# BrByte/brb_framework

Measured on AMD Instinct MI355X. Metric: GiB/s (device-resident) + Mrecords/s over 1500B buffers at 1/2/4/8 MI355X, higher is better.
Workload: dtype u32

## Files before the change

brb_framework_amd/__init__.py:

```python
from .crypto import (
    BATCH_ALL_DEVICES,
    BATCH_DROPPED,
    TRANSFORM_DROPPED,
    TestOption,
    test_option,
    async_fault_check,
    BATCH_ASYNC,
    BATCH_DEVICE,
    BATCH_HOST,
    BRB_BLOWFISH_CTX,
    BRB_MD5_CTX,
    BRB_RC4_State,
    RC4_STATE_BYTES,
    RC4MD5_HEADER,
    BrbSha1Ctx,
    LIB_PATH,
    CRYPTO_FUNC_RC4,
    CRYPTO_FUNC_RC4_MD5,
    OP_READ,
    OP_WRITE,
    TransformBatcher,
    HostRegion,
    BATCHER_ZERO_COPY,
    BATCHER_PIPELINED,
# ... 54 lines not shown
    sha1_final_batch,
    md5_update_segments_batch,
    sha1_update_segments_batch,
    md5_update_segments_lower_batch,
    md5_lower_text_batch,
    MD5_CTX_BYTES,
    SHA1_CTX_BYTES,
    md5_ctx_init,
    md5_ctx_update,
    md5_ctx_update_lower,
    md5_ctx_final,
    sha1_ctx_init,
    sha1_ctx_update,
    sha1_ctx_final,
    fixed_route,
    FIXED_ROUTE_LANE_A4,
    FIXED_ROUTE_LANE_ANY,
    FIXED_ROUTE_LINE,
    FIXED_ROUTE_VAR_LINE,
    FIXED_ROUTE_DMA_TICKET,
    FIXED_ROUTE_B64R_8,
    FIXED_ROUTE_B64R_4,
    FIXED_ROUTE_B64,
    FIXED_ROUTE_DMA_SHORT,
)

__all__ = [
    "BATCH_ASYNC", "BATCH_DEVICE", "BATCH_HOST", "BRB_BLOWFISH_CTX", "BRB_MD5_CTX", "BrbSha1Ctx",
    "LIB_PATH", "blowfish_ctx_bytes", "blowfish_decrypt_batch", "blowfish_encrypt_batch",
    "blowfish_init", "exported_symbols", "gpu_available", "lib", "md5_batch", "md5_batch_fixed",
    "sha1_batch", "sha1_batch_fixed", "BRB_RC4_State", "RC4_STATE_BYTES", "RC4MD5_HEADER", "rc4_crypt_batch",
    "rc4_init", "rc4_state_bytes", "rc4_states", "rc4md5_frame_batch", "rc4md5_open_batch", "rc4_crypt_list_batch",
    "rc4md5_frame_list_batch", "rc4md5_open_list_batch", "BATCHER_CONN_LISTS",
    "rc4_mixed_list_batch", "BATCHER_MIXED", "RC4_KIND_CRYPT", "RC4_KIND_FRAME", "RC4_KIND_OPEN", "membuf_decrypt",
    "membuf_encrypt", "membuf_key", "membuf_span", "md5_batch_segments", "metadata_pack_batch", "metadata_unpack_batch", "metadata_unpack_items_batch", "METADATA_INFO_DTYPE", "base64_decode_batch",
    "base64_encode_batch", "CRYPTO_FUNC_RC4", "CRYPTO_FUNC_RC4_MD5", "OP_READ", "OP_WRITE", "TransformBatcher",
    "HostRegion", "BATCHER_ZERO_COPY", "BATCHER_PIPELINED", "BATCH_ALL_DEVICES", "device_count",
    "BATCH_DROPPED", "TRANSFORM_DROPPED", "BATCHER_ALL_DEVICES", "TestOption", "test_option", "async_fault_check",
    "rc4_init_batch", "blowfish_init_batch", "pack_keys", "unpack_keys", "BLOWFISH_CTX_BYTES",
    "blowfish_contexts", "blowfish_encrypt_batch_keyed", "blowfish_decrypt_batch_keyed", "membuf_encrypt_batch",
    "membuf_decrypt_batch", "md5_init_batch", "md5_update_batch", "md5_final_batch", "sha1_init_batch",
    "sha1_update_batch", "sha1_final_batch", "md5_update_segments_batch", "sha1_update_segments_batch",
    "md5_update_segments_lower_batch", "md5_lower_text_batch", "md5_ctx_update_lower", "MD5_CTX_BYTES", "SHA1_CTX_BYTES",
    "md5_ctx_init", "md5_ctx_update", "md5_ctx_final", "sha1_ctx_init", "sha1_ctx_update", "sha1_ctx_final",
    "fixed_route", "FIXED_ROUTE_LANE_A4", "FIXED_ROUTE_LANE_ANY", "FIXED_ROUTE_LINE", "FIXED_ROUTE_VAR_LINE",
    "FIXED_ROUTE_DMA_TICKET", "FIXED_ROUTE_B64R_8", "FIXED_ROUTE_B64R_4", "FIXED_ROUTE_B64", "FIXED_ROUTE_DMA_SHORT",
]
```

brb_framework_amd/crypto.py:

```python
from __future__ import annotations

import ctypes
import os
import subprocess

import numpy as np

HERE = os.path.dirname(os.path.abspath(__file__))
LIB_PATH = os.environ.get("BRB_CRYPTO_LIB") or os.path.join(HERE, "libbrb_crypto_gpu.so")
HEADER_PATH = os.path.join(os.path.dirname(HERE), "include", "brb_crypto.h")

BATCH_HOST = 0x0
BATCH_DEVICE = 0x1
BATCH_ASYNC = 0x2
BATCH_ALL_DEVICES = 0x4
BATCH_DROPPED = -2
BATCH_PARTIAL = -3
BATCH_FAULT = -4
TRANSFORM_DROPPED = -1

u8p = ctypes.POINTER(ctypes.c_uint8)
ulp = ctypes.POINTER(ctypes.c_ulong)


# ... 163 lines not shown
     [ctypes.c_void_p, ctypes.c_uint32, ctypes.c_int, ctypes.c_void_p, ctypes.c_int]),
    ("BRB_TransformBatcherEnableBatchAlgo", ctypes.c_int,
     [ctypes.c_void_p, ctypes.c_void_p, ctypes.c_uint64, ctypes.c_void_p, ctypes.c_void_p, ctypes.c_void_p,
      ctypes.c_void_p]),
    ("BRB_TransformBatcherDisable", ctypes.c_int, [ctypes.c_void_p, ctypes.c_uint32]),
    ("BRB_TransformBatcherRead", ctypes.c_int, [ctypes.c_void_p, ctypes.c_uint32, ctypes.c_void_p, ctypes.c_uint32]),
    ("BRB_TransformBatcherWrite", ctypes.c_int,
     [ctypes.c_void_p, ctypes.c_uint32, ctypes.c_void_p, ctypes.c_uint32, ctypes.c_uint64]),
    ("BRB_TransformBatcherFlush", ctypes.c_int64, [ctypes.c_void_p, ctypes.c_void_p, ctypes.c_void_p]),
    ("BRB_TransformBatcherFlushAsync", ctypes.c_int64, [ctypes.c_void_p, ctypes.c_void_p, ctypes.c_void_p]),
    ("BRB_TransformBatcherGetState", ctypes.c_int,
     [ctypes.c_void_p, ctypes.c_uint32, ctypes.c_int, ctypes.POINTER(BRB_RC4_State)]),
    ("BRB_TransformBatcherInjectFault", ctypes.c_int, [ctypes.c_void_p, ctypes.c_int]),
    ("BRB_CryptoGPU_TestOption", ctypes.c_int, [ctypes.c_char_p, ctypes.c_int, ctypes.POINTER(ctypes.c_int)]),
    ("BRB_CryptoGPU_TestFixedRoute", ctypes.c_int, [ctypes.c_uint64, ctypes.c_uint32]),
    ("BRB_CryptoGPU_HostRegister", ctypes.c_int, [ctypes.c_void_p, ctypes.c_uint64]),
    ("BRB_CryptoGPU_HostUnregister", ctypes.c_int, [ctypes.c_void_p]),
    ("BRB_CryptoGPU_Available", ctypes.c_int, []),
    ("BRB_CryptoGPU_DeviceCount", ctypes.c_int, []),
    ("BRB_CryptoGPU_SetDevice", ctypes.c_int, [ctypes.c_int]),
    ("BRB_CryptoGPU_GetDevice", ctypes.c_int, []),
    ("BRB_CryptoGPU_ThreadCleanup", None, []),
    ("BRB_CryptoGPU_LastError", ctypes.c_char_p, []),
    ("BRB_CryptoGPU_AsyncFaultCheck", ctypes.c_int, []),
    ("BRB_CryptoGPU_Version", ctypes.c_char_p, []),
]


def lib() -> ctypes.CDLL:
    global _LIB
# ... 52 lines not shown
    def __enter__(self):
        self.old = test_option(self.name, self.value)
        return self

    def __exit__(self, *exc):
        test_option(self.name, self.old)
        return False


(FIXED_ROUTE_LANE_A4, FIXED_ROUTE_LANE_ANY, FIXED_ROUTE_LINE, FIXED_ROUTE_VAR_LINE, FIXED_ROUTE_DMA_TICKET,
 FIXED_ROUTE_B64R_8, FIXED_ROUTE_B64R_4, FIXED_ROUTE_B64, FIXED_ROUTE_DMA_SHORT) = range(9)


def fixed_route(addr: int, rec_len: int) -> int:
    return lib().BRB_CryptoGPU_TestFixedRoute(int(addr), int(rec_len))


def _check(rc: int, what: str) -> None:
    if rc != 1:
        msg = lib().BRB_CryptoGPU_LastError().decode(errors="replace")
        raise RuntimeError(f"{what} returned {rc}: {msg}")


def _is_torch(x) -> bool:
    return type(x).__module__.startswith("torch")


def _ptr(x) -> int:
    if x is None:
        return 0
# ... 782 lines not shown
```

brb_framework_amd/csrc/gpu/api_runtime.hip:

```cpp
#include <hip/hip_runtime.h>

#include <algorithm>
#include <atomic>
#include <cstdarg>
#include <cstdio>
#include <cstring>
#include <mutex>
#include <string>
#include <vector>

#include "brb_crypto.h"
#include "api_util.h"
#include "fixed_route.h"
#include "host_pipe.h"
#include "pair_fault.h"
#include "test_options.h"

namespace brb_api {

thread_local std::string t_err;

void clear_err()
{
    t_err.clear();
}

void set_err(const char *fmt, ...)
{
    char buf[512];
    va_list ap;
    va_start(ap, fmt);
// ... 301 lines not shown
            }
            const int prev = brb_opt::g_opt[k.opt].exchange(value, std::memory_order_relaxed);
            if (old)
                *old = prev;
            return BRB_BATCH_OK;
        }
    set_err("unknown test option '%s'", name);
    return BRB_BATCH_BADARG;
}

int BRB_CryptoGPU_TestFixedRoute(uint64_t data_addr, uint32_t rec_len)
{
    return brb_digest::fixed_route(uintptr_t(data_addr), rec_len);
}

}
```

brb_framework_amd/csrc/gpu/digest_var_line.h:

```cpp
#pragma once

#include "byte_stream.h"
#include "digest_line.h"
#include "test_options.h"

namespace brb_digest {

template <class Alg>
BRB_DEV typename Alg::State digest_lane(const uint8_t *a, uint64_t len)
{
    typename Alg::State st = Alg::iv();
    brb_io::BlockSrc src;
    src.init(a, len);
    uint32_t w[16];
    for (uint64_t b = 0; b < (len >> 6); ++b) {
        src.fetch(w);
        Alg::compress(st, w);
    }
    src.fetch(w);
    brb_io::add_marker(w, len);
    Alg::finish(st, w, uint32_t(len & 63), len);
    return st;
}

// ... 9 lines not shown
    for (int m = 32; m >= 1; m >>= 1) {
        const uint64_t o = __shfl_xor(v, m, 64);
        v = o < v ? o : v;
    }
    return v;
}

BRB_DEV uint64_t wave_max64(uint64_t v)
{
#pragma unroll
    for (int m = 32; m >= 1; m >>= 1) {
        const uint64_t o = __shfl_xor(v, m, 64);
        v = o > v ? o : v;
    }
    return v;
}

constexpr uint32_t kSortCG = 4;
constexpr uint32_t kSortNB = 8;

BRB_DEV uint64_t sorted_record(uint64_t g, uint32_t lane, const uint32_t *__restrict__ lens, uint64_t n_rec,
                               uint32_t *scratch)
{
    const uint64_t cg = (g / kSortCG) * kSortCG;
    const uint64_t c0 = cg * 64;
    const uint64_t left = (n_rec + 63) / 64 - cg;
    const uint32_t pc = left < kSortCG ? uint32_t(left) : kSortCG;
    const uint32_t j = uint32_t((g % kSortCG + g / gridDim.x) % pc);
    uint32_t it[kSortCG];
    bool ok[kSortCG];
// ... 75 lines not shown
        return uint64_t(blockIdx.x) + uint64_t(tk) * gridDim.x;
    };
    uint64_t g = uint64_t(blockIdx.x) + uint64_t(wv) * gridDim.x;
    if (g >= n_groups)
        return;
    const uint32_t my_off = wv * 2 * SLOT;
    const uint32_t lds0 = uint32_t(reinterpret_cast<uintptr_t>(ring)) + my_off;
    const uint64_t dbase = reinterpret_cast<uint64_t>(data);
    auto swz = [](uint32_t row) { return (row >> 1) & 7; };

    struct Grp {
        uint64_t a;
        uint64_t r;
        uint32_t len;
        uint32_t K;
        bool line;
        brb_dma::v4i rs;
        uint32_t vq[8];
        uint32_t lq[8];
    };
    const uint64_t first_sorted = brb_first_sorted;
    auto record_of = [&](uint64_t g) -> uint64_t {
        if (SORT && g >= first_sorted && g < n_groups)
            return sorted_record(g, lane, lens, n_rec, sort_scratch + wv * (64 * kSortCG));
        return g * 64 + lane < n_rec ? g * 64 + lane : ~uint64_t(0);
    };
    auto setup = [&](uint64_t g, uint64_t rec, Grp &G) {
        const uint64_t r = rec != ~uint64_t(0) ? rec : uniform64(g * 64);
        G.r = rec;
        G.a = dbase + (FIXED ? r * rec_len : offs[r]);
        G.len = FIXED ? rec_len : (rec != ~uint64_t(0) ? lens[r] : 0u);
        const uint64_t line = G.a & ~uint64_t(127);
        const uint32_t lines = G.len ? uint32_t(((G.a & 127) + G.len + 127) >> 7) : 0u;
        const uint32_t nblk = (G.len >> 6) + ((G.len & 63) ? 1u : 0u);
        const uint64_t lo = uniform64(wave_min64(G.len ? line : ~uint64_t(0)));
        const uint64_t hi = uniform64(wave_max64(G.len ? line + 128 * uint64_t(lines) : 0));
        G.K = __builtin_amdgcn_readfirstlane(uint32_t(wave_max64((nblk + 1) >> 1)));
        G.line = hi > lo && hi - lo < (uint64_t(1) << 31) - (uint64_t(1) << 16);
        const uint64_t base = lo - 4096;
        const uint64_t left = hi - base;
        G.rs.x = __builtin_amdgcn_readfirstlane(int(uint32_t(base)));
        G.rs.y = __builtin_amdgcn_readfirstlane(int(uint32_t(base >> 32) & 0xFFFF));
        G.rs.z = __builtin_amdgcn_readfirstlane(int(left > 0x7FFFFFFFull ? 0x7FFFFFFFu : uint32_t(left)));
        G.rs.w = 0x00020000;
        const uint32_t rel = uint32_t(line - lo);
        const uint32_t l3 = lane >> 3;
        const uint32_t g0 = 16u * ((lane & 7) ^ (l3 >> 1));
#pragma unroll
        for (int q = 0; q < 8; q++) {
            const int src = int(8 * q + l3) * 4;
            const uint32_t rrel = uint32_t(__builtin_amdgcn_ds_bpermute(src, int(rel)));
            G.lq[q] = uint32_t(__builtin_amdgcn_ds_bpermute(src, int(lines)));
            G.vq[q] = (rrel | (q & 1 ? g0 ^ 64u : g0)) + (4096u - 1024u * (q & 3));
        }
    };
    auto issue = [&](Grp &G, uint32_t m, uint32_t slot, bool keep_l2 = false) {
        const uint32_t lm = lds0 + slot * SLOT;
        uint32_t v[8];
#pragma unroll
        for (int q = 0; q < 8; q++)
            v[q] = m < G.lq[q] ? G.vq[q] : OOB;
        uint32_t keep;
#define BRB_VLINE_DMA8(POL)                                                                     \
        asm volatile("s_mov_b32 %0, m0\n\t"                                                    \
                     "s_mov_b32 m0, %10\n\t"                                                   \
                     "s_nop 0\n\t"                                                             \
                     "buffer_load_dwordx4 %1, %9, 0 offen " POL "lds\n\t"                      \
                     "buffer_load_dwordx4 %2, %9, 0 offen offset:1024 " POL "lds\n\t"          \
                     "buffer_load_dwordx4 %3, %9, 0 offen offset:2048 " POL "lds\n\t"          \
                     "buffer_load_dwordx4 %4, %9, 0 offen offset:3072 " POL "lds\n\t"          \
                     "s_mov_b32 m0, %11\n\t"                                                   \
                     "s_nop 0\n\t"                                                             \
                     "buffer_load_dwordx4 %5, %9, 0 offen " POL "lds\n\t"                      \
                     "buffer_load_dwordx4 %6, %9, 0 offen offset:1024 " POL "lds\n\t"          \
                     "buffer_load_dwordx4 %7, %9, 0 offen offset:2048 " POL "lds\n\t"          \
                     "buffer_load_dwordx4 %8, %9, 0 offen offset:3072 " POL "lds\n\t"          \
// ... 15 lines not shown
        G.rs.z = z;
    };
    auto start = [&](Grp &G) {
        if (G.line) {
            issue(G, 0, 0, FIXED);
            issue(G, 1, 1, FIXED);
        }
    };

    uint32_t ae[33], ao[33];
    auto win_setup = [&](const Grp &G) {
        const uint32_t sh4 = uint32_t(G.a) & 124u;
        const uint32_t fr = (my_off + lane * 128) | (swz(lane) << 4);
#pragma unroll
        for (uint32_t i = 0; i < 33; i++) {
            const uint32_t q4 = sh4 + 4 * i;
            ae[i] = ((q4 & 124u) ^ fr) | ((q4 & 128u) << 6);
            ao[i] = ae[i] ^ SLOT;
            asm volatile("" : "+v"(ao[i]));
        }
    };
    uint32_t w0[16], w1[16];
    auto read_window = [&](const uint32_t (&ad)[33], uint32_t fb) {
        uint32_t d[33];
#pragma unroll
        for (int i = 0; i < 33; i++)
            d[i] = *reinterpret_cast<const uint32_t *>(ring + ad[i]);
        __builtin_amdgcn_s_waitcnt(0xC07F);
#pragma unroll
        for (int i = 0; i < 16; i++) {
            w0[i] = __builtin_amdgcn_alignbit(d[i + 1], d[i], fb);
            w1[i] = __builtin_amdgcn_alignbit(d[i + 17], d[i + 16], fb);
// ... 7 lines not shown
    for (;;) {
        const uint64_t gn = take();
        const uint64_t rn = record_of(gn);
        const uint64_t r = G.r;
        typename Alg::State st;
        if (!G.line) {
            st = digest_lane<Alg>(reinterpret_cast<const uint8_t *>(G.a), G.len);
            if (gn < n_groups) {
                setup(gn, rn, Gn);
                start(Gn);
            }
        } else {
            win_setup(G);
            const uint32_t fb = (uint32_t(G.a) & 3u) * 8u;
            const uint32_t nfull = G.len >> 6, t = G.len & 63;
            const uint32_t tb = t ? nfull : 0xFFFFFFFFu;
            uint32_t wt[16];
#pragma unroll
            for (int i = 0; i < 16; i++)
                wt[i] = 0;
            st = Alg::iv();
            const uint32_t K = G.K;
            auto step = [&](uint32_t k, const uint32_t (&ad)[33], uint32_t refill_slot) {
                brb_dma::wait_vmcnt<0>();
                read_window(ad, fb);
                if (k < K) {
                    issue(G, k + 1, refill_slot);
                } else if (gn < n_groups) {
                    setup(gn, rn, Gn);
                    start(Gn);
                }
                const uint32_t b = 2 * k - 2;
                if (b < nfull)
                    Alg::compress(st, w0);
                if (b + 1 < nfull)
                    Alg::compress(st, w1);
                if (__builtin_amdgcn_ballot_w64(tb - b < 2) != 0) {
#pragma unroll
                    for (int i = 0; i < 16; i++)
                        wt[i] = tb == b ? w0[i] : tb == b + 1 ? w1[i] : wt[i];
                }
            };
            if (K == 0) {
                brb_dma::wait_vmcnt<0>();
                if (gn < n_groups) {
                    setup(gn, rn, Gn);
                    start(Gn);
                }
            }
            for (uint32_t k = 1; k <= K; k += 2) {
                step(k, ae, 0);
                if (k == K)
                    break;
                step(k + 1, ao, 1);
            }
            if (t == 0) {
                Alg::pad_only(st, G.len);
            } else {
#pragma unroll
                for (uint32_t i = 0; i < 16; i++) {
                    const uint32_t o = 4 * i;
                    const uint32_t keep = t > o ? (t - o < 4 ? t - o : 4) : 0;
                    uint32_t v = keep == 4 ? wt[i] : wt[i] & ((1u << (8 * keep)) - 1u);
                    if (t >= o && t < o + 4)
                        v |= 0x80u << (8 * (t - o));
                    wt[i] = v;
                }
                Alg::finish(st, wt, t, G.len);
            }
        }
        if (r != ~uint64_t(0))
            Alg::template store<OUT_ALIGNED>(out, r, st);
        g = gn;
        if (g >= n_groups)
            break;
        G = Gn;
    }
}

template <class Alg>
hipError_t launch_var_line(const uint8_t *data, const uint64_t *offs, const uint32_t *lens, uint64_t n_rec, uint8_t *out,
                           bool out_al, hipStream_t s)
{
// ... 37 lines not shown
```

brb_framework_amd/csrc/gpu/md5_device.h:

```cpp
#pragma once

#include "brb_gpu_common.h"

#define BRB_MD5_F1(x, y, z) ((z) ^ ((x) & ((y) ^ (z))))
#define BRB_MD5_F2(x, y, z) ((y) ^ ((z) & ((x) ^ (y))))
#define BRB_MD5_F3(x, y, z) __builtin_amdgcn_bitop3_b32((x), (y), (z), 0x96)
#define BRB_MD5_F4(x, y, z) ((y) ^ ((x) | ~(z)))
#define BRB_MD5_STEP(F, a, b, c, d, m, k, s) (a) = (b) + rotl<s>((a) + F((b), (c), (d)) + ((m) + (k)))

struct Md5State {
    uint32_t a, b, c, d;
};

BRB_DEV Md5State md5_iv()
{
    return Md5State{0x67452301u, 0xefcdab89u, 0x98badcfeu, 0x10325476u};
}

#define BRB_MD5_STEP3X(a, b, c, d, m, k, s)                                               \
    do {                                                                                 \
        const uint32_t x_ = (a) + (m) + (k), cd_ = (c) ^ (d);                            \
        uint32_t f_;                                                                     \
        asm("v_xad_u32 %0, %1, %2, %3" : "=v"(f_) : "v"(b), "v"(cd_), "v"(x_));          \
        (a) = (b) + rotl<s>(f_);                                                         \
    } while (0)

template <bool XAD = true>
BRB_DEV void md5_compress(Md5State &st, const uint32_t (&m)[16])
{
    uint32_t a = st.a, b = st.b, c = st.c, d = st.d;

    BRB_MD5_STEP(BRB_MD5_F1, a, b, c, d, m[0], 0xd76aa478u, 7);
    BRB_MD5_STEP(BRB_MD5_F1, d, a, b, c, m[1], 0xe8c7b756u, 12);
    BRB_MD5_STEP(BRB_MD5_F1, c, d, a, b, m[2], 0x242070dbu, 17);
    BRB_MD5_STEP(BRB_MD5_F1, b, c, d, a, m[3], 0xc1bdceeeu, 22);
    BRB_MD5_STEP(BRB_MD5_F1, a, b, c, d, m[4], 0xf57c0fafu, 7);
    BRB_MD5_STEP(BRB_MD5_F1, d, a, b, c, m[5], 0x4787c62au, 12);
    BRB_MD5_STEP(BRB_MD5_F1, c, d, a, b, m[6], 0xa8304613u, 17);
    BRB_MD5_STEP(BRB_MD5_F1, b, c, d, a, m[7], 0xfd469501u, 22);
    BRB_MD5_STEP(BRB_MD5_F1, a, b, c, d, m[8], 0x698098d8u, 7);
    BRB_MD5_STEP(BRB_MD5_F1, d, a, b, c, m[9], 0x8b44f7afu, 12);
    BRB_MD5_STEP(BRB_MD5_F1, c, d, a, b, m[10], 0xffff5bb1u, 17);
    BRB_MD5_STEP(BRB_MD5_F1, b, c, d, a, m[11], 0x895cd7beu, 22);
    BRB_MD5_STEP(BRB_MD5_F1, a, b, c, d, m[12], 0x6b901122u, 7);
    BRB_MD5_STEP(BRB_MD5_F1, d, a, b, c, m[13], 0xfd987193u, 12);
// ... 5 lines not shown
    BRB_MD5_STEP(BRB_MD5_F2, c, d, a, b, m[11], 0x265e5a51u, 14);
    BRB_MD5_STEP(BRB_MD5_F2, b, c, d, a, m[0], 0xe9b6c7aau, 20);
    BRB_MD5_STEP(BRB_MD5_F2, a, b, c, d, m[5], 0xd62f105du, 5);
    BRB_MD5_STEP(BRB_MD5_F2, d, a, b, c, m[10], 0x02441453u, 9);
    BRB_MD5_STEP(BRB_MD5_F2, c, d, a, b, m[15], 0xd8a1e681u, 14);
    BRB_MD5_STEP(BRB_MD5_F2, b, c, d, a, m[4], 0xe7d3fbc8u, 20);
    BRB_MD5_STEP(BRB_MD5_F2, a, b, c, d, m[9], 0x21e1cde6u, 5);
    BRB_MD5_STEP(BRB_MD5_F2, d, a, b, c, m[14], 0xc33707d6u, 9);
    BRB_MD5_STEP(BRB_MD5_F2, c, d, a, b, m[3], 0xf4d50d87u, 14);
    BRB_MD5_STEP(BRB_MD5_F2, b, c, d, a, m[8], 0x455a14edu, 20);
    BRB_MD5_STEP(BRB_MD5_F2, a, b, c, d, m[13], 0xa9e3e905u, 5);
    BRB_MD5_STEP(BRB_MD5_F2, d, a, b, c, m[2], 0xfcefa3f8u, 9);
    BRB_MD5_STEP(BRB_MD5_F2, c, d, a, b, m[7], 0x676f02d9u, 14);
    BRB_MD5_STEP(BRB_MD5_F2, b, c, d, a, m[12], 0x8d2a4c8au, 20);

    if constexpr (XAD) BRB_MD5_STEP3X(a, b, c, d, m[5], 0xfffa3942u, 4); else BRB_MD5_STEP(BRB_MD5_F3, a, b, c, d, m[5], 0xfffa3942u, 4);
    if constexpr (XAD) BRB_MD5_STEP3X(d, a, b, c, m[8], 0x8771f681u, 11); else BRB_MD5_STEP(BRB_MD5_F3, d, a, b, c, m[8], 0x8771f681u, 11);
    if constexpr (XAD) BRB_MD5_STEP3X(c, d, a, b, m[11], 0x6d9d6122u, 16); else BRB_MD5_STEP(BRB_MD5_F3, c, d, a, b, m[11], 0x6d9d6122u, 16);
    if constexpr (XAD) BRB_MD5_STEP3X(b, c, d, a, m[14], 0xfde5380cu, 23); else BRB_MD5_STEP(BRB_MD5_F3, b, c, d, a, m[14], 0xfde5380cu, 23);
    if constexpr (XAD) BRB_MD5_STEP3X(a, b, c, d, m[1], 0xa4beea44u, 4); else BRB_MD5_STEP(BRB_MD5_F3, a, b, c, d, m[1], 0xa4beea44u, 4);
    if constexpr (XAD) BRB_MD5_STEP3X(d, a, b, c, m[4], 0x4bdecfa9u, 11); else BRB_MD5_STEP(BRB_MD5_F3, d, a, b, c, m[4], 0x4bdecfa9u, 11);
    if constexpr (XAD) BRB_MD5_STEP3X(c, d, a, b, m[7], 0xf6bb4b60u, 16); else BRB_MD5_STEP(BRB_MD5_F3, c, d, a, b, m[7], 0xf6bb4b60u, 16);
    if constexpr (XAD) BRB_MD5_STEP3X(b, c, d, a, m[10], 0xbebfbc70u, 23); else BRB_MD5_STEP(BRB_MD5_F3, b, c, d, a, m[10], 0xbebfbc70u, 23);
    if constexpr (XAD) BRB_MD5_STEP3X(a, b, c, d, m[13], 0x289b7ec6u, 4); else BRB_MD5_STEP(BRB_MD5_F3, a, b, c, d, m[13], 0x289b7ec6u, 4);
    if constexpr (XAD) BRB_MD5_STEP3X(d, a, b, c, m[0], 0xeaa127fau, 11); else BRB_MD5_STEP(BRB_MD5_F3, d, a, b, c, m[0], 0xeaa127fau, 11);
    if constexpr (XAD) BRB_MD5_STEP3X(c, d, a, b, m[3], 0xd4ef3085u, 16); else BRB_MD5_STEP(BRB_MD5_F3, c, d, a, b, m[3], 0xd4ef3085u, 16);
    if constexpr (XAD) BRB_MD5_STEP3X(b, c, d, a, m[6], 0x04881d05u, 23); else BRB_MD5_STEP(BRB_MD5_F3, b, c, d, a, m[6], 0x04881d05u, 23);
    if constexpr (XAD) BRB_MD5_STEP3X(a, b, c, d, m[9], 0xd9d4d039u, 4); else BRB_MD5_STEP(BRB_MD5_F3, a, b, c, d, m[9], 0xd9d4d039u, 4);
    if constexpr (XAD) BRB_MD5_STEP3X(d, a, b, c, m[12], 0xe6db99e5u, 11); else BRB_MD5_STEP(BRB_MD5_F3, d, a, b, c, m[12], 0xe6db99e5u, 11);
    if constexpr (XAD) BRB_MD5_STEP3X(c, d, a, b, m[15], 0x1fa27cf8u, 16); else BRB_MD5_STEP(BRB_MD5_F3, c, d, a, b, m[15], 0x1fa27cf8u, 16);
    if constexpr (XAD) BRB_MD5_STEP3X(b, c, d, a, m[2], 0xc4ac5665u, 23); else BRB_MD5_STEP(BRB_MD5_F3, b, c, d, a, m[2], 0xc4ac5665u, 23);

    BRB_MD5_STEP(BRB_MD5_F4, a, b, c, d, m[0], 0xf4292244u, 6);
    BRB_MD5_STEP(BRB_MD5_F4, d, a, b, c, m[7], 0x432aff97u, 10);
    BRB_MD5_STEP(BRB_MD5_F4, c, d, a, b, m[14], 0xab9423a7u, 15);
    BRB_MD5_STEP(BRB_MD5_F4, b, c, d, a, m[5], 0xfc93a039u, 21);
    BRB_MD5_STEP(BRB_MD5_F4, a, b, c, d, m[12], 0x655b59c3u, 6);
    BRB_MD5_STEP(BRB_MD5_F4, d, a, b, c, m[3], 0x8f0ccc92u, 10);
    BRB_MD5_STEP(BRB_MD5_F4, c, d, a, b, m[10], 0xffeff47du, 15);
    BRB_MD5_STEP(BRB_MD5_F4, b, c, d, a, m[1], 0x85845dd1u, 21);
    BRB_MD5_STEP(BRB_MD5_F4, a, b, c, d, m[8], 0x6fa87e4fu, 6);
    BRB_MD5_STEP(BRB_MD5_F4, d, a, b, c, m[15], 0xfe2ce6e0u, 10);
    BRB_MD5_STEP(BRB_MD5_F4, c, d, a, b, m[6], 0xa3014314u, 15);
    BRB_MD5_STEP(BRB_MD5_F4, b, c, d, a, m[13], 0x4e0811a1u, 21);
    BRB_MD5_STEP(BRB_MD5_F4, a, b, c, d, m[4], 0xf7537e82u, 6);
    BRB_MD5_STEP(BRB_MD5_F4, d, a, b, c, m[11], 0xbd3af235u, 10);
// ... 24 lines not shown
};

BRB_DEV void md5_finish(Md5State &st, uint32_t (&w)[16], uint32_t t, uint64_t total_len)
{
    if (t >= 56) {
        md5_compress(st, w);
#pragma unroll
        for (int i = 0; i < 14; i++)
            w[i] = 0;
    }
    w[14] = uint32_t(total_len << 3);
    w[15] = uint32_t(total_len >> 29);
    md5_compress(st, w);
}

BRB_DEV void md5_pad_only(Md5State &st, uint64_t total_len)
{
    uint32_t w[16] = {0x80u};
    w[14] = uint32_t(total_len << 3);
    w[15] = uint32_t(total_len >> 29);
    md5_compress<false>(st, w);
}
```

brb_framework_amd/csrc/gpu/md5_kernels.hip:

```cpp
#include "brb_kernels.h"
#include "byte_stream.h"
#include "digest_dma.h"
#include "digest_var_line.h"
#include "md5_device.h"

namespace {

struct Md5Alg;

struct Out16 {
    template <bool ALIGNED>
    static BRB_DEV void store(uint8_t *out, uint64_t r, const Md5State &st)
    {
        const uint4 v = make_uint4(st.a, st.b, st.c, st.d);
        if (ALIGNED)
            reinterpret_cast<uint4 *>(out)[r] = v;
        else
            __builtin_memcpy(out + 16 * r, &v, 16);
    }
};

struct Md5Alg {
    using State = Md5State;
    static BRB_DEV State iv() { return md5_iv(); }
    static BRB_DEV void compress(State &st, uint32_t (&w)[16]) { md5_compress(st, w); }
    static BRB_DEV void finish(State &st, uint32_t (&w)[16], uint32_t t, uint64_t len) { md5_finish(st, w, t, len); }
    static BRB_DEV void pad_only(State &st, uint64_t len) { md5_pad_only(st, len); }
    template <bool ALIGNED>
    static BRB_DEV void store(uint8_t *out, uint64_t r, const State &st) { Out16::store<ALIGNED>(out, r, st); }
};

template <int BLOCK, bool OUT_ALIGNED>
__global__ __launch_bounds__(BLOCK) void md5_fixed_a4_kernel(const uint8_t *__restrict__ data, uint32_t rec_len,
                                                              uint64_t n_rec, uint8_t *__restrict__ out)
{
    const uint64_t r = uint64_t(blockIdx.x) * BLOCK + threadIdx.x;
    if (r >= n_rec)
        return;
    const uint8_t *p = data + r * rec_len;
    const uint32_t nfull = rec_len >> 6;
    Md5State st = md5_iv();
// ... 106 lines not shown
```

brb_framework_amd/csrc/gpu/sha1_device.h:

```cpp
#pragma once

#include "brb_gpu_common.h"

struct Sha1State {
    uint32_t a, b, c, d, e;
};

BRB_DEV Sha1State sha1_iv()
{
    return Sha1State{0x67452301u, 0xEFCDAB89u, 0x98BADCFEu, 0x10325476u, 0xC3D2E1F0u};
}

#define BRB_SHA1_CH(b, c, d) __builtin_amdgcn_bitop3_b32((b), (c), (d), 0xCA)
#define BRB_SHA1_PAR(b, c, d) __builtin_amdgcn_bitop3_b32((b), (c), (d), 0x96)
#define BRB_SHA1_MAJ(b, c, d) __builtin_amdgcn_bitop3_b32((b), (c), (d), 0xE8)
#define BRB_SHA1_W(i) \
    (w[(i) & 15] = rotl<1>(__builtin_amdgcn_bitop3_b32(w[((i) + 13) & 15], w[((i) + 8) & 15], w[((i) + 2) & 15], 0x96) ^ w[(i) & 15]))
#define BRB_SHA1_R(F, K, v, x, y, z, u, wi)                    \
    do {                                                       \
        (u) += F((x), (y), (z)) + (wi) + (K) + rotl<5>(v);     \
        (x) = rotl<30>(x);                                     \
    } while (0)

BRB_DEV void sha1_compress(Sha1State &st, uint32_t (&w)[16])
// ... 33 lines not shown
{
#pragma unroll
    for (int i = 0; i < 16; i++)
        w[i] = __builtin_bswap32(w[i]);
    if (t >= 56) {
        sha1_compress(st, w);
#pragma unroll
        for (int i = 0; i < 14; i++)
            w[i] = 0;
    }
    w[14] = uint32_t(len >> 29) + (len >= (uint64_t(1) << 29) ? 1u : 0u);
    w[15] = uint32_t(len << 3);
    sha1_compress(st, w);
}

BRB_DEV void sha1_pad_only(Sha1State &st, uint64_t len)
{
    uint32_t w[16] = {0x80000000u};
    w[14] = uint32_t(len >> 29) + (len >= (uint64_t(1) << 29) ? 1u : 0u);
    w[15] = uint32_t(len << 3);
    sha1_compress(st, w);
}
```

brb_framework_amd/csrc/gpu/sha1_kernels.hip:

```cpp
#include "brb_kernels.h"
#include "byte_stream.h"
#include "digest_dma.h"
#include "digest_var_line.h"
#include "sha1_device.h"

namespace {

template <bool ALIGNED>
BRB_DEV void store20(uint8_t *out, uint64_t r, const Sha1State &st)
{
    const uint32_t v[5] = {__builtin_bswap32(st.a), __builtin_bswap32(st.b), __builtin_bswap32(st.c),
                           __builtin_bswap32(st.d), __builtin_bswap32(st.e)};
    uint8_t *o = out + 20 * r;
    if (ALIGNED) {
        uint32_t *o32 = reinterpret_cast<uint32_t *>(o);
#pragma unroll
        for (int i = 0; i < 5; i++)
            o32[i] = v[i];
    } else {
        __builtin_memcpy(o, v, 20);
    }
}

struct Sha1Alg {
    using State = Sha1State;
    static BRB_DEV State iv() { return sha1_iv(); }
    static BRB_DEV void compress(State &st, uint32_t (&w)[16])
    {
#pragma unroll
        for (int i = 0; i < 16; i++)
            w[i] = __builtin_bswap32(w[i]);
        sha1_compress(st, w);
    }
    static BRB_DEV void finish(State &st, uint32_t (&w)[16], uint32_t t, uint64_t len) { sha1_finish(st, w, t, len); }
    static BRB_DEV void pad_only(State &st, uint64_t len) { sha1_pad_only(st, len); }
    template <bool ALIGNED>
    static BRB_DEV void store(uint8_t *out, uint64_t r, const State &st) { store20<ALIGNED>(out, r, st); }
};

template <int BLOCK, bool OUT_ALIGNED>
__global__ __launch_bounds__(BLOCK) void sha1_fixed_a4_kernel(const uint8_t *__restrict__ data, uint32_t rec_len,
                                                               uint64_t n_rec, uint8_t *__restrict__ out)
{
    const uint64_t r = uint64_t(blockIdx.x) * BLOCK + threadIdx.x;
    if (r >= n_rec)
        return;
    const uint8_t *p = data + r * rec_len;
    const uint32_t nfull = rec_len >> 6;
    Sha1State st = sha1_iv();
// ... 112 lines not shown
```

include/brb_crypto.h:

```cpp
#ifndef BRB_CRYPTO_H
#define BRB_CRYPTO_H

#include <stddef.h>
#include <stdint.h>

#ifdef __cplusplus
extern "C" {
#endif

#ifndef LIBBRB_DATA_H_

#define MD5_DIGEST_LENGTH 16

typedef struct _BRB_MD5_CTX {
    uint32_t buf[4];
    uint32_t bytes[2];
    uint32_t in[16];
    unsigned char digest[16];
    unsigned char string[64];
} BRB_MD5_CTX;

void BRB_MD5Init(BRB_MD5_CTX *ctx);
void BRB_MD5UpdateBig(BRB_MD5_CTX *ctx, const void *_buf, unsigned long len);
void BRB_MD5Update(BRB_MD5_CTX *ctx, const void *_buf, unsigned long len);
// ... 243 lines not shown
const char *BRB_CryptoGPU_LastError(void);
int BRB_CryptoGPU_AsyncFaultCheck(void);
int BRB_CryptoGPU_HostRegister(void *p, uint64_t len);
int BRB_CryptoGPU_HostUnregister(void *p);
int BRB_CryptoGPU_TestOption(const char *name, int value, int *old);
#define BRB_FIXED_ROUTE_LANE_A4    0
#define BRB_FIXED_ROUTE_LANE_ANY   1
#define BRB_FIXED_ROUTE_LINE       2
#define BRB_FIXED_ROUTE_VAR_LINE   3
#define BRB_FIXED_ROUTE_DMA_TICKET 4
#define BRB_FIXED_ROUTE_B64R_8     5
#define BRB_FIXED_ROUTE_B64R_4     6
#define BRB_FIXED_ROUTE_B64        7
#define BRB_FIXED_ROUTE_DMA_SHORT  8
int BRB_CryptoGPU_TestFixedRoute(uint64_t data_addr, uint32_t rec_len);
const char *BRB_CryptoGPU_Version(void);

#ifdef __cplusplus
}
#endif
#endif
```

Measured before the change: 4578.

## Rework var-line LDS window layout, skip bounds masks, simplify tail handling

```diff
diff --git a/brb_framework_amd/__init__.py b/brb_framework_amd/__init__.py
--- a/brb_framework_amd/__init__.py
+++ b/brb_framework_amd/__init__.py
@@ -92,6 +92,7 @@
     sha1_ctx_update,
     sha1_ctx_final,
     fixed_route,
+    var_line_layout,
     FIXED_ROUTE_LANE_A4,
     FIXED_ROUTE_LANE_ANY,
     FIXED_ROUTE_LINE,
@@ -121,6 +122,6 @@
     "sha1_update_batch", "sha1_final_batch", "md5_update_segments_batch", "sha1_update_segments_batch",
     "md5_update_segments_lower_batch", "md5_lower_text_batch", "md5_ctx_update_lower", "MD5_CTX_BYTES", "SHA1_CTX_BYTES",
     "md5_ctx_init", "md5_ctx_update", "md5_ctx_final", "sha1_ctx_init", "sha1_ctx_update", "sha1_ctx_final",
-    "fixed_route", "FIXED_ROUTE_LANE_A4", "FIXED_ROUTE_LANE_ANY", "FIXED_ROUTE_LINE", "FIXED_ROUTE_VAR_LINE",
+    "fixed_route", "var_line_layout", "FIXED_ROUTE_LANE_A4", "FIXED_ROUTE_LANE_ANY", "FIXED_ROUTE_LINE", "FIXED_ROUTE_VAR_LINE",
     "FIXED_ROUTE_DMA_TICKET", "FIXED_ROUTE_B64R_8", "FIXED_ROUTE_B64R_4", "FIXED_ROUTE_B64", "FIXED_ROUTE_DMA_SHORT",
 ]
diff --git a/brb_framework_amd/crypto.py b/brb_framework_amd/crypto.py
--- a/brb_framework_amd/crypto.py
+++ b/brb_framework_amd/crypto.py
@@ -201,6 +201,7 @@
     ("BRB_TransformBatcherInjectFault", ctypes.c_int, [ctypes.c_void_p, ctypes.c_int]),
     ("BRB_CryptoGPU_TestOption", ctypes.c_int, [ctypes.c_char_p, ctypes.c_int, ctypes.POINTER(ctypes.c_int)]),
     ("BRB_CryptoGPU_TestFixedRoute", ctypes.c_int, [ctypes.c_uint64, ctypes.c_uint32]),
+    ("BRB_CryptoGPU_TestVarLineLayout", ctypes.c_int, [ctypes.c_void_p] * 4),
     ("BRB_CryptoGPU_HostRegister", ctypes.c_int, [ctypes.c_void_p, ctypes.c_uint64]),
     ("BRB_CryptoGPU_HostUnregister", ctypes.c_int, [ctypes.c_void_p]),
     ("BRB_CryptoGPU_Available", ctypes.c_int, []),
@@ -283,6 +284,16 @@
 
 def fixed_route(addr: int, rec_len: int) -> int:
     return lib().BRB_CryptoGPU_TestFixedRoute(int(addr), int(rec_len))
+
+
+def var_line_layout(sh):
+    sh = np.ascontiguousarray(sh, dtype=np.uint32)
+    if sh.shape != (64,):
+        raise ValueError("sh holds one dword shift per lane of a 64-record group")
+    rho, src, win = np.zeros(64, np.uint32), np.zeros((64, 8), np.uint32), np.zeros((64, 33), np.uint32)
+    _check(lib().BRB_CryptoGPU_TestVarLineLayout(sh.ctypes.data, rho.ctypes.data, src.ctypes.data, win.ctypes.data),
+           "BRB_CryptoGPU_TestVarLineLayout")
+    return rho, src, win
 
 
 def _check(rc: int, what: str) -> None:
diff --git a/brb_framework_amd/csrc/gpu/api_runtime.hip b/brb_framework_amd/csrc/gpu/api_runtime.hip
--- a/brb_framework_amd/csrc/gpu/api_runtime.hip
+++ b/brb_framework_amd/csrc/gpu/api_runtime.hip
@@ -15,6 +15,7 @@
 #include "host_pipe.h"
 #include "pair_fault.h"
 #include "test_options.h"
+#include "var_line_layout.h"
 
 namespace brb_api {
 
@@ -346,4 +347,26 @@
     return brb_digest::fixed_route(uintptr_t(data_addr), rec_len);
 }
 
-}
+int BRB_CryptoGPU_TestVarLineLayout(const uint32_t *sh, uint32_t *rho, uint32_t *src, uint32_t *win)
+{
+    if (!sh || !rho || !src || !win) {
+        set_err("BRB_CryptoGPU_TestVarLineLayout: NULL argument");
+        return BRB_BATCH_BADARG;
+    }
+    for (uint32_t l = 0; l < 64; l++)
+        if (sh[l] > 31) {
+            set_err("BRB_CryptoGPU_TestVarLineLayout: sh[%u] = %u is no dword shift (0..31)", l, sh[l]);
+            return BRB_BATCH_BADARG;
+        }
+    for (uint32_t l = 0; l < 64; l++) {
+        rho[l] = brb_vl::rot(sh[l], brb_vl::rank_of(sh, l));
+        for (uint32_t p = 0; p < 8; p++)
+            src[8 * l + p] = brb_vl::src_granule(p, rho[l]);
+        const uint32_t key = brb_vl::win_key(sh[l], rho[l]);
+        for (uint32_t i = 0; i < 33; i++)
+            win[33 * l + i] = brb_vl::win_off(key, i);
+    }
+    return BRB_BATCH_OK;
+}
+
+}
diff --git a/brb_framework_amd/csrc/gpu/digest_var_line.h b/brb_framework_amd/csrc/gpu/digest_var_line.h
--- a/brb_framework_amd/csrc/gpu/digest_var_line.h
+++ b/brb_framework_amd/csrc/gpu/digest_var_line.h
@@ -3,6 +3,7 @@
 #include "byte_stream.h"
 #include "digest_line.h"
 #include "test_options.h"
+#include "var_line_layout.h"
 
 namespace brb_digest {
 
@@ -47,6 +48,16 @@
         v = o > v ? o : v;
     }
     return v;
+}
+
+BRB_DEV void wave_max_min32(uint32_t &a, uint32_t &b)
+{
+#pragma unroll
+    for (int m = 32; m >= 1; m >>= 1) {
+        const uint32_t oa = uint32_t(__shfl_xor(int(a), m, 64)), ob = uint32_t(__shfl_xor(int(b), m, 64));
+        a = oa > a ? oa : a;
+        b = ob < b ? ob : b;
+    }
 }
 
 constexpr uint32_t kSortCG = 4;
@@ -152,6 +163,8 @@
         uint64_t r;
         uint32_t len;
         uint32_t K;
+        uint32_t lmin;
+        uint32_t wkey;
         bool line;
         brb_dma::v4i rs;
         uint32_t vq[8];
@@ -173,7 +186,10 @@
         const uint32_t nblk = (G.len >> 6) + ((G.len & 63) ? 1u : 0u);
         const uint64_t lo = uniform64(wave_min64(G.len ? line : ~uint64_t(0)));
         const uint64_t hi = uniform64(wave_max64(G.len ? line + 128 * uint64_t(lines) : 0));
-        G.K = __builtin_amdgcn_readfirstlane(uint32_t(wave_max64((nblk + 1) >> 1)));
+        uint32_t kmax = (nblk + 1) >> 1, lmin = lines;
+        wave_max_min32(kmax, lmin);
+        G.K = __builtin_amdgcn_readfirstlane(kmax);
+        G.lmin = __builtin_amdgcn_readfirstlane(lmin);
         G.line = hi > lo && hi - lo < (uint64_t(1) << 31) - (uint64_t(1) << 16);
         const uint64_t base = lo - 4096;
         const uint64_t left = hi - base;
@@ -181,23 +197,46 @@
         G.rs.y = __builtin_amdgcn_readfirstlane(int(uint32_t(base >> 32) & 0xFFFF));
         G.rs.z = __builtin_amdgcn_readfirstlane(int(left > 0x7FFFFFFFull ? 0x7FFFFFFFu : uint32_t(left)));
         G.rs.w = 0x00020000;
-        const uint32_t rel = uint32_t(line - lo);
+        uint32_t rel = uint32_t(line - lo);
         const uint32_t l3 = lane >> 3;
+        if constexpr (!FIXED) {
+            const uint32_t sh = (uint32_t(G.a) >> 2) & 31u;
+            uint32_t rank = 0;
+#pragma unroll
+            for (uint32_t c = 0; c < 4; c++) {
+                const uint64_t m = __builtin_amdgcn_ballot_w64((sh & 3u) == c);
+                const uint32_t below_lo = __builtin_amdgcn_mbcnt_lo(uint32_t(m), 0u);
+                const uint32_t below_hi = __builtin_amdgcn_mbcnt_hi(uint32_t(m >> 32), 0u);
+                rank = (sh & 3u) == c ? (lane < 32 ? below_lo : below_hi) : rank;
+            }
+            const uint32_t rho = brb_vl::rot(sh, rank);
+            G.wkey = brb_vl::win_key(sh, rho);
+            rel |= ((8u - rho) & 7u) << 4;
+        }
         const uint32_t g0 = 16u * ((lane & 7) ^ (l3 >> 1));
 #pragma unroll
         for (int q = 0; q < 8; q++) {
             const int src = int(8 * q + l3) * 4;
             const uint32_t rrel = uint32_t(__builtin_amdgcn_ds_bpermute(src, int(rel)));
             G.lq[q] = uint32_t(__builtin_amdgcn_ds_bpermute(src, int(lines)));
-            G.vq[q] = (rrel | (q & 1 ? g0 ^ 64u : g0)) + (4096u - 1024u * (q & 3));
+            if constexpr (FIXED)
+                G.vq[q] = (rrel | (q & 1 ? g0 ^ 64u : g0)) + (4096u - 1024u * (q & 3));
+            else
+                G.vq[q] = ((rrel & ~0x70u) | ((rrel + 16u * (lane & 7)) & 0x70u)) + (4096u - 1024u * (q & 3));
         }
     };
     auto issue = [&](Grp &G, uint32_t m, uint32_t slot, bool keep_l2 = false) {
         const uint32_t lm = lds0 + slot * SLOT;
         uint32_t v[8];
-#pragma unroll
-        for (int q = 0; q < 8; q++)
-            v[q] = m < G.lq[q] ? G.vq[q] : OOB;
+        if (m < G.lmin) {
+#pragma unroll
+            for (int q = 0; q < 8; q++)
+                v[q] = G.vq[q];
+        } else {
+#pragma unroll
+            for (int q = 0; q < 8; q++)
+                v[q] = m < G.lq[q] ? G.vq[q] : OOB;
+        }
         uint32_t keep;
 #define BRB_VLINE_DMA8(POL)                                                                     \
         asm volatile("s_mov_b32 %0, m0\n\t"                                                    \
@@ -243,8 +282,12 @@
         const uint32_t fr = (my_off + lane * 128) | (swz(lane) << 4);
 #pragma unroll
         for (uint32_t i = 0; i < 33; i++) {
-            const uint32_t q4 = sh4 + 4 * i;
-            ae[i] = ((q4 & 124u) ^ fr) | ((q4 & 128u) << 6);
+            if constexpr (FIXED) {
+                const uint32_t q4 = sh4 + 4 * i;
+                ae[i] = ((q4 & 124u) ^ fr) | ((q4 & 128u) << 6);
+            } else {
+                ae[i] = brb_vl::win_off(G.wkey, i) | (my_off + lane * 128);
+            }
             ao[i] = ae[i] ^ SLOT;
             asm volatile("" : "+v"(ao[i]));
         }
@@ -282,16 +325,13 @@
             win_setup(G);
             const uint32_t fb = (uint32_t(G.a) & 3u) * 8u;
             const uint32_t nfull = G.len >> 6, t = G.len & 63;
-            const uint32_t tb = t ? nfull : 0xFFFFFFFFu;
-            uint32_t wt[16];
-#pragma unroll
-            for (int i = 0; i < 16; i++)
-                wt[i] = 0;
+            const uint32_t kl = (nfull + (t ? 1u : 0u) + 1) >> 1;
             st = Alg::iv();
             const uint32_t K = G.K;
             auto step = [&](uint32_t k, const uint32_t (&ad)[33], uint32_t refill_slot) {
                 brb_dma::wait_vmcnt<0>();
-                read_window(ad, fb);
+                if (k <= kl)
+                    read_window(ad, fb);
                 if (k < K) {
                     issue(G, k + 1, refill_slot);
                 } else if (gn < n_groups) {
@@ -303,11 +343,6 @@
                     Alg::compress(st, w0);
                 if (b + 1 < nfull)
                     Alg::compress(st, w1);
-                if (__builtin_amdgcn_ballot_w64(tb - b < 2) != 0) {
-#pragma unroll
-                    for (int i = 0; i < 16; i++)
-                        wt[i] = tb == b ? w0[i] : tb == b + 1 ? w1[i] : wt[i];
-                }
             };
             if (K == 0) {
                 brb_dma::wait_vmcnt<0>();
@@ -322,11 +357,13 @@
                     break;
                 step(k + 1, ao, 1);
             }
-            if (t == 0) {
+            if (FIXED ? t == 0 : __builtin_amdgcn_ballot_w64(t != 0) == 0) {
                 Alg::pad_only(st, G.len);
             } else {
+                uint32_t wt[16];
 #pragma unroll
                 for (uint32_t i = 0; i < 16; i++) {
+                    wt[i] = (nfull & 1) ? w1[i] : w0[i];
                     const uint32_t o = 4 * i;
                     const uint32_t keep = t > o ? (t - o < 4 ? t - o : 4) : 0;
                     uint32_t v = keep == 4 ? wt[i] : wt[i] & ((1u << (8 * keep)) - 1u);
@@ -334,7 +371,10 @@
                         v |= 0x80u << (8 * (t - o));
                     wt[i] = v;
                 }
-                Alg::finish(st, wt, t, G.len);
+                if constexpr (FIXED)
+                    Alg::finish(st, wt, t, G.len);
+                else
+                    Alg::finish_mixed(st, wt, t, G.len);
             }
         }
         if (r != ~uint64_t(0))
diff --git a/brb_framework_amd/csrc/gpu/md5_device.h b/brb_framework_amd/csrc/gpu/md5_device.h
--- a/brb_framework_amd/csrc/gpu/md5_device.h
+++ b/brb_framework_amd/csrc/gpu/md5_device.h
@@ -17,6 +17,21 @@
     return Md5State{0x67452301u, 0xefcdab89u, 0x98badcfeu, 0x10325476u};
 }
 
+#define BRB_MD5_STEP3A(a, b, c, d, m, k, s, bc)                                          \
+    do {                                                                                 \
+        const uint32_t x_ = (a) + (m) + (k);                                             \
+        uint32_t f_;                                                                     \
+        (bc) = (b) ^ (c);                                                                \
+        asm("v_xad_u32 %0, %1, %2, %3" : "=v"(f_) : "v"(bc), "v"(d), "v"(x_));           \
+        (a) = (b) + rotl<s>(f_);                                                         \
+    } while (0)
+#define BRB_MD5_STEP3B(a, b, c, d, m, k, s, bc)                                          \
+    do {                                                                                 \
+        const uint32_t x_ = (a) + (m) + (k);                                             \
+        uint32_t f_;                                                                     \
+        asm("v_xad_u32 %0, %1, %2, %3" : "=v"(f_) : "v"(b), "v"(bc), "v"(x_));           \
+        (a) = (b) + rotl<s>(f_);                                                         \
+    } while (0)
 #define BRB_MD5_STEP3X(a, b, c, d, m, k, s)                                               \
     do {                                                                                 \
         const uint32_t x_ = (a) + (m) + (k), cd_ = (c) ^ (d);                            \
@@ -29,6 +44,7 @@
 BRB_DEV void md5_compress(Md5State &st, const uint32_t (&m)[16])
 {
     uint32_t a = st.a, b = st.b, c = st.c, d = st.d;
+    [[maybe_unused]] uint32_t bc;
 
     BRB_MD5_STEP(BRB_MD5_F1, a, b, c, d, m[0], 0xd76aa478u, 7);
     BRB_MD5_STEP(BRB_MD5_F1, d, a, b, c, m[1], 0xe8c7b756u, 12);
@@ -64,22 +80,22 @@
     BRB_MD5_STEP(BRB_MD5_F2, c, d, a, b, m[7], 0x676f02d9u, 14);
     BRB_MD5_STEP(BRB_MD5_F2, b, c, d, a, m[12], 0x8d2a4c8au, 20);
 
-    if constexpr (XAD) BRB_MD5_STEP3X(a, b, c, d, m[5], 0xfffa3942u, 4); else BRB_MD5_STEP(BRB_MD5_F3, a, b, c, d, m[5], 0xfffa3942u, 4);
-    if constexpr (XAD) BRB_MD5_STEP3X(d, a, b, c, m[8], 0x8771f681u, 11); else BRB_MD5_STEP(BRB_MD5_F3, d, a, b, c, m[8], 0x8771f681u, 11);
-    if constexpr (XAD) BRB_MD5_STEP3X(c, d, a, b, m[11], 0x6d9d6122u, 16); else BRB_MD5_STEP(BRB_MD5_F3, c, d, a, b, m[11], 0x6d9d6122u, 16);
-    if constexpr (XAD) BRB_MD5_STEP3X(b, c, d, a, m[14], 0xfde5380cu, 23); else BRB_MD5_STEP(BRB_MD5_F3, b, c, d, a, m[14], 0xfde5380cu, 23);
-    if constexpr (XAD) BRB_MD5_STEP3X(a, b, c, d, m[1], 0xa4beea44u, 4); else BRB_MD5_STEP(BRB_MD5_F3, a, b, c, d, m[1], 0xa4beea44u, 4);
-    if constexpr (XAD) BRB_MD5_STEP3X(d, a, b, c, m[4], 0x4bdecfa9u, 11); else BRB_MD5_STEP(BRB_MD5_F3, d, a, b, c, m[4], 0x4bdecfa9u, 11);
-    if constexpr (XAD) BRB_MD5_STEP3X(c, d, a, b, m[7], 0xf6bb4b60u, 16); else BRB_MD5_STEP(BRB_MD5_F3, c, d, a, b, m[7], 0xf6bb4b60u, 16);
-    if constexpr (XAD) BRB_MD5_STEP3X(b, c, d, a, m[10], 0xbebfbc70u, 23); else BRB_MD5_STEP(BRB_MD5_F3, b, c, d, a, m[10], 0xbebfbc70u, 23);
-    if constexpr (XAD) BRB_MD5_STEP3X(a, b, c, d, m[13], 0x289b7ec6u, 4); else BRB_MD5_STEP(BRB_MD5_F3, a, b, c, d, m[13], 0x289b7ec6u, 4);
-    if constexpr (XAD) BRB_MD5_STEP3X(d, a, b, c, m[0], 0xeaa127fau, 11); else BRB_MD5_STEP(BRB_MD5_F3, d, a, b, c, m[0], 0xeaa127fau, 11);
-    if constexpr (XAD) BRB_MD5_STEP3X(c, d, a, b, m[3], 0xd4ef3085u, 16); else BRB_MD5_STEP(BRB_MD5_F3, c, d, a, b, m[3], 0xd4ef3085u, 16);
-    if constexpr (XAD) BRB_MD5_STEP3X(b, c, d, a, m[6], 0x04881d05u, 23); else BRB_MD5_STEP(BRB_MD5_F3, b, c, d, a, m[6], 0x04881d05u, 23);
-    if constexpr (XAD) BRB_MD5_STEP3X(a, b, c, d, m[9], 0xd9d4d039u, 4); else BRB_MD5_STEP(BRB_MD5_F3, a, b, c, d, m[9], 0xd9d4d039u, 4);
-    if constexpr (XAD) BRB_MD5_STEP3X(d, a, b, c, m[12], 0xe6db99e5u, 11); else BRB_MD5_STEP(BRB_MD5_F3, d, a, b, c, m[12], 0xe6db99e5u, 11);
-    if constexpr (XAD) BRB_MD5_STEP3X(c, d, a, b, m[15], 0x1fa27cf8u, 16); else BRB_MD5_STEP(BRB_MD5_F3, c, d, a, b, m[15], 0x1fa27cf8u, 16);
-    if constexpr (XAD) BRB_MD5_STEP3X(b, c, d, a, m[2], 0xc4ac5665u, 23); else BRB_MD5_STEP(BRB_MD5_F3, b, c, d, a, m[2], 0xc4ac5665u, 23);
+    if constexpr (XAD) BRB_MD5_STEP3A(a, b, c, d, m[5], 0xfffa3942u, 4, bc); else BRB_MD5_STEP(BRB_MD5_F3, a, b, c, d, m[5], 0xfffa3942u, 4);
+    if constexpr (XAD) BRB_MD5_STEP3B(d, a, b, c, m[8], 0x8771f681u, 11, bc); else BRB_MD5_STEP(BRB_MD5_F3, d, a, b, c, m[8], 0x8771f681u, 11);
+    if constexpr (XAD) BRB_MD5_STEP3A(c, d, a, b, m[11], 0x6d9d6122u, 16, bc); else BRB_MD5_STEP(BRB_MD5_F3, c, d, a, b, m[11], 0x6d9d6122u, 16);
+    if constexpr (XAD) BRB_MD5_STEP3B(b, c, d, a, m[14], 0xfde5380cu, 23, bc); else BRB_MD5_STEP(BRB_MD5_F3, b, c, d, a, m[14], 0xfde5380cu, 23);
+    if constexpr (XAD) BRB_MD5_STEP3A(a, b, c, d, m[1], 0xa4beea44u, 4, bc); else BRB_MD5_STEP(BRB_MD5_F3, a, b, c, d, m[1], 0xa4beea44u, 4);
+    if constexpr (XAD) BRB_MD5_STEP3B(d, a, b, c, m[4], 0x4bdecfa9u, 11, bc); else BRB_MD5_STEP(BRB_MD5_F3, d, a, b, c, m[4], 0x4bdecfa9u, 11);
+    if constexpr (XAD) BRB_MD5_STEP3A(c, d, a, b, m[7], 0xf6bb4b60u, 16, bc); else BRB_MD5_STEP(BRB_MD5_F3, c, d, a, b, m[7], 0xf6bb4b60u, 16);
+    if constexpr (XAD) BRB_MD5_STEP3B(b, c, d, a, m[10], 0xbebfbc70u, 23, bc); else BRB_MD5_STEP(BRB_MD5_F3, b, c, d, a, m[10], 0xbebfbc70u, 23);
+    if constexpr (XAD) BRB_MD5_STEP3A(a, b, c, d, m[13], 0x289b7ec6u, 4, bc); else BRB_MD5_STEP(BRB_MD5_F3, a, b, c, d, m[13], 0x289b7ec6u, 4);
+    if constexpr (XAD) BRB_MD5_STEP3B(d, a, b, c, m[0], 0xeaa127fau, 11, bc); else BRB_MD5_STEP(BRB_MD5_F3, d, a, b, c, m[0], 0xeaa127fau, 11);
+    if constexpr (XAD) BRB_MD5_STEP3A(c, d, a, b, m[3], 0xd4ef3085u, 16, bc); else BRB_MD5_STEP(BRB_MD5_F3, c, d, a, b, m[3], 0xd4ef3085u, 16);
+    if constexpr (XAD) BRB_MD5_STEP3B(b, c, d, a, m[6], 0x04881d05u, 23, bc); else BRB_MD5_STEP(BRB_MD5_F3, b, c, d, a, m[6], 0x04881d05u, 23);
+    if constexpr (XAD) BRB_MD5_STEP3A(a, b, c, d, m[9], 0xd9d4d039u, 4, bc); else BRB_MD5_STEP(BRB_MD5_F3, a, b, c, d, m[9], 0xd9d4d039u, 4);
+    if constexpr (XAD) BRB_MD5_STEP3B(d, a, b, c, m[12], 0xe6db99e5u, 11, bc); else BRB_MD5_STEP(BRB_MD5_F3, d, a, b, c, m[12], 0xe6db99e5u, 11);
+    if constexpr (XAD) BRB_MD5_STEP3A(c, d, a, b, m[15], 0x1fa27cf8u, 16, bc); else BRB_MD5_STEP(BRB_MD5_F3, c, d, a, b, m[15], 0x1fa27cf8u, 16);
+    if constexpr (XAD) BRB_MD5_STEP3B(b, c, d, a, m[2], 0xc4ac5665u, 23, bc); else BRB_MD5_STEP(BRB_MD5_F3, b, c, d, a, m[2], 0xc4ac5665u, 23);
 
     BRB_MD5_STEP(BRB_MD5_F4, a, b, c, d, m[0], 0xf4292244u, 6);
     BRB_MD5_STEP(BRB_MD5_F4, d, a, b, c, m[7], 0x432aff97u, 10);
@@ -134,6 +150,21 @@
     md5_compress(st, w);
 }
 
+BRB_DEV void md5_finish_mixed(Md5State &st, uint32_t (&w)[16], uint32_t t, uint64_t total_len)
+{
+    if (t < 56) {
+        w[14] = uint32_t(total_len << 3);
+        w[15] = uint32_t(total_len >> 29);
+    }
+    md5_compress(st, w);
+    if (t >= 56) {
+        uint32_t z[16] = {0};
+        z[14] = uint32_t(total_len << 3);
+        z[15] = uint32_t(total_len >> 29);
+        md5_compress<false>(st, z);
+    }
+}
+
 BRB_DEV void md5_pad_only(Md5State &st, uint64_t total_len)
 {
     uint32_t w[16] = {0x80u};
diff --git a/brb_framework_amd/csrc/gpu/md5_kernels.hip b/brb_framework_amd/csrc/gpu/md5_kernels.hip
--- a/brb_framework_amd/csrc/gpu/md5_kernels.hip
+++ b/brb_framework_amd/csrc/gpu/md5_kernels.hip
@@ -25,6 +25,7 @@
     static BRB_DEV State iv() { return md5_iv(); }
     static BRB_DEV void compress(State &st, uint32_t (&w)[16]) { md5_compress(st, w); }
     static BRB_DEV void finish(State &st, uint32_t (&w)[16], uint32_t t, uint64_t len) { md5_finish(st, w, t, len); }
+    static BRB_DEV void finish_mixed(State &st, uint32_t (&w)[16], uint32_t t, uint64_t len) { md5_finish_mixed(st, w, t, len); }
     static BRB_DEV void pad_only(State &st, uint64_t len) { md5_pad_only(st, len); }
     template <bool ALIGNED>
     static BRB_DEV void store(uint8_t *out, uint64_t r, const State &st) { Out16::store<ALIGNED>(out, r, st); }
diff --git a/brb_framework_amd/csrc/gpu/sha1_device.h b/brb_framework_amd/csrc/gpu/sha1_device.h
--- a/brb_framework_amd/csrc/gpu/sha1_device.h
+++ b/brb_framework_amd/csrc/gpu/sha1_device.h
@@ -71,6 +71,25 @@
     sha1_compress(st, w);
 }
 
+BRB_DEV void sha1_finish_mixed(Sha1State &st, uint32_t (&w)[16], uint32_t t, uint64_t len)
+{
+    const uint32_t hi = uint32_t(len >> 29) + (len >= (uint64_t(1) << 29) ? 1u : 0u), lo = uint32_t(len << 3);
+#pragma unroll
+    for (int i = 0; i < 16; i++)
+        w[i] = __builtin_bswap32(w[i]);
+    if (t < 56) {
+        w[14] = hi;
+        w[15] = lo;
+    }
+    sha1_compress(st, w);
+    if (t >= 56) {
+        uint32_t z[16] = {0};
+        z[14] = hi;
+        z[15] = lo;
+        sha1_compress(st, z);
+    }
+}
+
 BRB_DEV void sha1_pad_only(Sha1State &st, uint64_t len)
 {
     uint32_t w[16] = {0x80000000u};
diff --git a/brb_framework_amd/csrc/gpu/sha1_kernels.hip b/brb_framework_amd/csrc/gpu/sha1_kernels.hip
--- a/brb_framework_amd/csrc/gpu/sha1_kernels.hip
+++ b/brb_framework_amd/csrc/gpu/sha1_kernels.hip
@@ -33,6 +33,7 @@
         sha1_compress(st, w);
     }
     static BRB_DEV void finish(State &st, uint32_t (&w)[16], uint32_t t, uint64_t len) { sha1_finish(st, w, t, len); }
+    static BRB_DEV void finish_mixed(State &st, uint32_t (&w)[16], uint32_t t, uint64_t len) { sha1_finish_mixed(st, w, t, len); }
     static BRB_DEV void pad_only(State &st, uint64_t len) { sha1_pad_only(st, len); }
     template <bool ALIGNED>
     static BRB_DEV void store(uint8_t *out, uint64_t r, const State &st) { store20<ALIGNED>(out, r, st); }
diff --git a/brb_framework_amd/csrc/gpu/var_line_layout.h b/brb_framework_amd/csrc/gpu/var_line_layout.h
--- /dev/null
+++ b/brb_framework_amd/csrc/gpu/var_line_layout.h
@@ -0,0 +1,41 @@
+#pragma once
+
+#include <stdint.h>
+
+#ifdef __HIPCC__
+#define BRB_VL_HD __host__ __device__ inline
+#else
+#define BRB_VL_HD inline
+#endif
+
+namespace brb_vl {
+
+inline uint32_t rank_of(const uint32_t *sh, uint32_t lane)
+{
+    uint32_t rank = 0;
+    for (uint32_t l = lane & 32u; l < lane; l++)
+        rank += (sh[l] & 3u) == (sh[lane] & 3u);
+    return rank;
+}
+
+BRB_VL_HD uint32_t rot(uint32_t sh, uint32_t rank)
+{
+    return (rank - (sh >> 2)) & 7u;
+}
+
+BRB_VL_HD uint32_t src_granule(uint32_t p, uint32_t rho)
+{
+    return (p - rho) & 7u;
+}
+
+BRB_VL_HD uint32_t win_key(uint32_t sh, uint32_t rho)
+{
+    return (sh << 8) | (((sh + 4u * rho) & 31u) << 2);
+}
+
+BRB_VL_HD uint32_t win_off(uint32_t key, uint32_t i)
+{
+    return (key + 260u * i) & 0x207Cu;
+}
+
+}
diff --git a/include/brb_crypto.h b/include/brb_crypto.h
--- a/include/brb_crypto.h
+++ b/include/brb_crypto.h
@@ -281,6 +281,7 @@
 #define BRB_FIXED_ROUTE_B64        7
 #define BRB_FIXED_ROUTE_DMA_SHORT  8
 int BRB_CryptoGPU_TestFixedRoute(uint64_t data_addr, uint32_t rec_len);
+int BRB_CryptoGPU_TestVarLineLayout(const uint32_t *sh, uint32_t *rho, uint32_t *src, uint32_t *win);
 const char *BRB_CryptoGPU_Version(void);
 
 #ifdef __cplusplus
```

After: 4634, median of 6. 1.01x the previous value.
